# facebookresearch/habitat-lab

Hardware: NVIDIA H100
Metric: DD-PPO learner frames/sec (ResNet18 RGB-D 256x256) (higher is better)
Workload: dtype bf16

## Files before the change

habitat-lab_b200/csrc/elementwise.cu:

```cuda
#include "common.cuh"
#include "wgmma.cuh"
#include <cooperative_groups.h>

namespace hb200 {
namespace cg = cooperative_groups;
using wg::cp_async16;
using wg::cp_async_commit;
using wg::cp_async_wait;
using wg::smem_u32;
void count_launch(int n);

static inline int grid_for(long long n, int bs) {
  long long g = (n + bs - 1) / bs;
  const long long cap = (long long)kNumSMs * 16;
  return (int)(g < 1 ? 1 : (g > cap ? cap : g));
}

template <bool HAS_RGB, bool HAS_DEPTH>
__device__ __forceinline__ void pooled4(const uint8_t* __restrict__ rgb, const float* __restrict__ depth,
                                        size_t row, int H, int W, int py, int px4, float rgb_scale,
                                        float (&out)[4][4]) {
#pragma unroll
  for (int p = 0; p < 4; ++p)
#pragma unroll
    for (int c = 0; c < 4; ++c) out[p][c] = 0.f;
  if (HAS_RGB) {
    const uint8_t* base = rgb + (row * H + 2 * py) * (size_t)W * 3 + (size_t)px4 * 8 * 3;
    uint8_t v[2][24];
#pragma unroll
    for (int r = 0; r < 2; ++r) {
      const uint2* src = reinterpret_cast<const uint2*>(base + (size_t)r * W * 3);
#pragma unroll
      for (int q = 0; q < 3; ++q) {
        const uint2 u = __ldg(src + q);
        *reinterpret_cast<uint2*>(&v[r][q * 8]) = u;
      }
    }
#pragma unroll
    for (int p = 0; p < 4; ++p)
#pragma unroll
      for (int c = 0; c < 3; ++c) {
        float s = __fmul_rn((float)v[0][(2 * p) * 3 + c], rgb_scale);
        s = __fadd_rn(s, __fmul_rn((float)v[0][(2 * p + 1) * 3 + c], rgb_scale));
        s = __fadd_rn(s, __fmul_rn((float)v[1][(2 * p) * 3 + c], rgb_scale));
        s = __fadd_rn(s, __fmul_rn((float)v[1][(2 * p + 1) * 3 + c], rgb_scale));
        out[p][c] = s * 0.25f;
      }
  }
  if (HAS_DEPTH) {
    const int dc = HAS_RGB ? 3 : 0;
    const float* base = depth + (row * H + 2 * py) * (size_t)W + (size_t)px4 * 8;
    float d[2][8];
#pragma unroll
    for (int r = 0; r < 2; ++r) {
      const float4* src = reinterpret_cast<const float4*>(base + (size_t)r * W);
      const float4 a = __ldg(src), b = __ldg(src + 1);
      d[r][0] = a.x; d[r][1] = a.y; d[r][2] = a.z; d[r][3] = a.w;
      d[r][4] = b.x; d[r][5] = b.y; d[r][6] = b.z; d[r][7] = b.w;
    }
#pragma unroll
    for (int p = 0; p < 4; ++p) {
      float s = __fadd_rn(d[0][2 * p], d[0][2 * p + 1]);
      s = __fadd_rn(s, d[1][2 * p]);
      s = __fadd_rn(s, d[1][2 * p + 1]);
      out[p][dc] = s * 0.25f;
    }
  }
}

template <bool HAS_RGB, bool HAS_DEPTH>
__global__ void __launch_bounds__(256)
prep_stats_kernel(const uint8_t* __restrict__ rgb, const float* __restrict__ depth,
                  const int32_t* __restrict__ frame_rows, int B, int H, int W, float rgb_scale,
                  double* __restrict__ stats) {
  __shared__ double red[32];
  const int Hp = H / 2, Wq = W / 8;
  const long long total = (long long)B * Hp * Wq;
  float s[4] = {0, 0, 0, 0}, q[4] = {0, 0, 0, 0};
  for (long long i = blockIdx.x * (long long)blockDim.x + threadIdx.x; i < total;
       i += (long long)gridDim.x * blockDim.x) {
    const int px4 = (int)(i % Wq);
    const long long t = i / Wq;
    const int py = (int)(t % Hp);
    const int f = (int)(t / Hp);
    float o[4][4];
    pooled4<HAS_RGB, HAS_DEPTH>(rgb, depth, (size_t)frame_rows[f], H, W, py, px4, rgb_scale, o);
#pragma unroll
    for (int p = 0; p < 4; ++p)
#pragma unroll
      for (int c = 0; c < 4; ++c) { s[c] += o[p][c]; q[c] = fmaf(o[p][c], o[p][c], q[c]); }
  }
#pragma unroll
  for (int c = 0; c < 4; ++c) {
    const double a = block_sum((double)s[c], red);
    const double b = block_sum((double)q[c], red);
    if (threadIdx.x == 0) { atomicAdd(&stats[c], a); atomicAdd(&stats[8 + c], b); }
  }
  if (blockIdx.x == 0 && threadIdx.x == 0) stats[16] = (double)B;
}

template <bool HAS_RGB, bool HAS_DEPTH, bool S2D>
__global__ void __launch_bounds__(256)
prep_apply_kernel(const uint8_t* __restrict__ rgb, const float* __restrict__ depth,
                  const int32_t* __restrict__ frame_rows, int B, int H, int W, float rgb_scale,
                  const float* __restrict__ scale_shift, act_t* __restrict__ out, grad_t* __restrict__ out2) {
  const int Hp = H / 2, Wq = W / 8;
  const long long total = (long long)B * Hp * Wq;
  float sc[4] = {1, 1, 1, 1}, sh[4] = {0, 0, 0, 0};
  if (scale_shift) {
#pragma unroll
    for (int c = 0; c < 4; ++c) { sc[c] = scale_shift[c]; sh[c] = scale_shift[8 + c]; }
  }
  const int C = (HAS_RGB ? 3 : 0) + (HAS_DEPTH ? 1 : 0);
  for (long long i = blockIdx.x * (long long)blockDim.x + threadIdx.x; i < total;
       i += (long long)gridDim.x * blockDim.x) {
    const int px4 = (int)(i % Wq);
    const long long t = i / Wq;
    const int py = (int)(t % Hp);
    const int f = (int)(t / Hp);
    float o[4][4];
    pooled4<HAS_RGB, HAS_DEPTH>(rgb, depth, (size_t)frame_rows[f], H, W, py, px4, rgb_scale, o);
    if (!S2D) {
      uint4* dst = reinterpret_cast<uint4*>(out + (((size_t)f * Hp + py) * (W / 2) + (size_t)px4 * 4) * 8);
#pragma unroll
      for (int p = 0; p < 4; ++p) {
        float v[8] = {0, 0, 0, 0, 0, 0, 0, 0};
#pragma unroll
        for (int c = 0; c < 4; ++c)
          if (c < C) v[c] = fmaf(o[p][c], sc[c], sh[c]);
        dst[p] = pack8a(v);
        if (out2) reinterpret_cast<uint4*>(out2 + (((size_t)f * Hp + py) * (W / 2) + (size_t)px4 * 4) * 8)[p] = pack8(v);
      }
    } else {
      const int i2 = py >> 1, dy = py & 1;
#pragma unroll
      for (int q = 0; q < 2; ++q) {
        float v[8];
#pragma unroll
        for (int dx = 0; dx < 2; ++dx)
#pragma unroll
          for (int c = 0; c < 4; ++c) v[dx * 4 + c] = (c < C) ? fmaf(o[2 * q + dx][c], sc[c], sh[c]) : 0.f;
        const size_t pix = ((size_t)f * (Hp / 2) + i2) * (W / 4) + (size_t)px4 * 2 + q;
        *reinterpret_cast<uint4*>(out + pix * 16 + dy * 8) = pack8a(v);
        if (out2) *reinterpret_cast<uint4*>(out2 + pix * 16 + dy * 8) = pack8(v);
      }
    }
  }
}

__global__ void prep_finalize_kernel(const double* __restrict__ stats, float* __restrict__ run_mean,
                                     float* __restrict__ run_var, float* __restrict__ run_count,
                                     float* __restrict__ scale_shift, int C, long long pix_per_frame,
                                     int update) {
  const int c = threadIdx.x;
  __shared__ float s_count;
  if (c == 0) s_count = run_count[0];
  __syncthreads();
  if (c < C) {
    float mean = run_mean[c], var = run_var[c];
    if (update) {
      const double frames = stats[16];
      const double n_el = frames * (double)pix_per_frame;
      const double nm = stats[c] / n_el;
      double nv = stats[8 + c] / n_el - nm * nm;
      if (nv < 0) nv = 0;
      const float count = s_count, new_count = (float)frames;
      const float new_mean = (float)nm, new_var = (float)nv;
      const float m_a = var * count, m_b = new_var * new_count;
      const float d = new_mean - mean;
      const float M2 = m_a + m_b + d * d * count * new_count / (count + new_count);
      var = M2 / (count + new_count);
      mean = (count * mean + new_count * new_mean) / (count + new_count);
      run_mean[c] = mean;
      run_var[c] = var;
    }
    const float inv = 1.0f / sqrtf(fmaxf(var, 1e-2f));
    scale_shift[c] = inv;
    scale_shift[8 + c] = -mean * inv;
  } else if (c < 8) {
    scale_shift[c] = 0.f;
    scale_shift[8 + c] = 0.f;
  }
  __syncthreads();
  if (c == 0 && update) run_count[0] = s_count + (float)stats[16];
}

struct GnP {
  const double* stats;
  const float* gamma;
  const float* beta;
  int C, G, lcpg;
  float inv_m, eps;
};

__device__ __forceinline__ void gn_coeffs(const GnP& p, int b, int c0, float (&mu)[8], float (&rs)[8]) {
  int prev = -1;
  float m = 0.f, r = 0.f;
#pragma unroll
  for (int e = 0; e < 8; ++e) {
    const int g = (c0 + e) >> p.lcpg;
    if (g != prev) {
      const double2 st = *reinterpret_cast<const double2*>(p.stats + ((size_t)b * p.G + g) * 2);
      const double md = st.x * (double)p.inv_m;
      m = (float)md;
      const float var = fmaxf((float)(st.y * (double)p.inv_m - md * md), 0.f);
      r = rsqrtf(var + p.eps);
      prev = g;
    }
    mu[e] = m;
    rs[e] = r;
  }
}
__device__ __forceinline__ void load8f(const float* __restrict__ p, float (&f)[8]) {
  const float4 a = __ldg(reinterpret_cast<const float4*>(p));
  const float4 b = __ldg(reinterpret_cast<const float4*>(p) + 1);
  f[0] = a.x; f[1] = a.y; f[2] = a.z; f[3] = a.w; f[4] = b.x; f[5] = b.y; f[6] = b.z; f[7] = b.w;
}

struct GnSlab {
  int b, vec, c0, pix0, pix1, npl, pl;
};
__device__ __forceinline__ GnSlab gn_slab(int C, int hw, int ppb) {
  GnSlab s;
  const int cv = C >> 3;
  const int slabs = (hw + ppb - 1) / ppb;
  s.b = blockIdx.x / slabs;
  const int slab = blockIdx.x - s.b * slabs;
  s.vec = threadIdx.x % cv;
  s.pl = threadIdx.x / cv;
  s.npl = blockDim.x / cv;
  s.c0 = s.vec << 3;
  s.pix0 = slab * ppb;
  s.pix1 = min(hw, s.pix0 + ppb);
  return s;
}

template <int OUT_F32>
__global__ void __launch_bounds__(256)
gn_apply_kernel(const act_t* __restrict__ y, GnP p, void* __restrict__ out, grad_t* __restrict__ out2, int B, int hw,
                int relu, int ppb) {
  const GnSlab t = gn_slab(p.C, hw, ppb);
  const int cv = p.C >> 3;
  float mu[8], rs[8], ga[8], be[8], sc[8], sh[8];
  gn_coeffs(p, t.b, t.c0, mu, rs);
  load8f(p.gamma + t.c0, ga);
  load8f(p.beta + t.c0, be);
#pragma unroll
  for (int e = 0; e < 8; ++e) { sc[e] = rs[e] * ga[e]; sh[e] = fmaf(-mu[e], sc[e], be[e]); }
  for (int pix = t.pix0 + t.pl; pix < t.pix1; pix += t.npl) {
    const size_t i = ((size_t)t.b * hw + pix) * cv + t.vec;
    float x[8];
    unpack8a(reinterpret_cast<const uint4*>(y)[i], x);
#pragma unroll
    for (int e = 0; e < 8; ++e) {
      const float z = fmaf(x[e], sc[e], sh[e]);
      x[e] = relu ? fmaxf(z, 0.f) : z;
    }
    if (OUT_F32 == 1) {
      float4* o = reinterpret_cast<float4*>(out) + 2 * i;
      o[0] = make_float4(x[0], x[1], x[2], x[3]);
      o[1] = make_float4(x[4], x[5], x[6], x[7]);
    } else if (OUT_F32 == 2) {
      float* o = reinterpret_cast<float*>(out) + (size_t)t.b * p.C * hw;
#pragma unroll
      for (int e = 0; e < 8; ++e) o[(size_t)(t.c0 + e) * hw + pix] = x[e];
    } else {
      reinterpret_cast<uint4*>(out)[i] = pack8a(x);
      if (out2) reinterpret_cast<uint4*>(out2)[i] = pack8(x);
    }
  }
}

__global__ void __launch_bounds__(256)
gn_residual_relu_kernel(const act_t* __restrict__ y, GnP p, const act_t* __restrict__ res,
                        GnP rp, int res_is_prenorm, act_t* __restrict__ out, grad_t* __restrict__ out2, int B, int hw,
                        int ppb) {
  const GnSlab t = gn_slab(p.C, hw, ppb);
  const int cv = p.C >> 3;
  float mu[8], rs[8], ga[8], be[8], sc[8], sh[8], rsc[8], rsh[8];
  gn_coeffs(p, t.b, t.c0, mu, rs);
  load8f(p.gamma + t.c0, ga);
  load8f(p.beta + t.c0, be);
#pragma unroll
  for (int e = 0; e < 8; ++e) { sc[e] = rs[e] * ga[e]; sh[e] = fmaf(-mu[e], sc[e], be[e]); rsc[e] = 1.f; rsh[e] = 0.f; }
  if (res_is_prenorm) {
    gn_coeffs(rp, t.b, t.c0, mu, rs);
    load8f(rp.gamma + t.c0, ga);
    load8f(rp.beta + t.c0, be);
#pragma unroll
    for (int e = 0; e < 8; ++e) { rsc[e] = rs[e] * ga[e]; rsh[e] = fmaf(-mu[e], rsc[e], be[e]); }
  }
  for (int pix = t.pix0 + t.pl; pix < t.pix1; pix += t.npl) {
    const size_t i = ((size_t)t.b * hw + pix) * cv + t.vec;
    float x[8], r[8];
    unpack8a(reinterpret_cast<const uint4*>(y)[i], x);
    unpack8a(reinterpret_cast<const uint4*>(res)[i], r);
#pragma unroll
    for (int e = 0; e < 8; ++e) x[e] = fmaxf(fmaf(x[e], sc[e], sh[e]) + fmaf(r[e], rsc[e], rsh[e]), 0.f);
    reinterpret_cast<uint4*>(out)[i] = pack8a(x);
    if (out2) reinterpret_cast<uint4*>(out2)[i] = pack8(x);
  }
}

__global__ void __launch_bounds__(256)
gn_relu_maxpool_kernel(const act_t* __restrict__ y, GnP p, act_t* __restrict__ out, grad_t* __restrict__ out2,
                       uint8_t* __restrict__ argmax, int B, int H, int W) {
  const int cv = p.C >> 3, Ho = (H + 1) / 2, Wo = (W + 1) / 2;
  const long long total = (long long)B * Ho * Wo * cv;
  for (long long i = blockIdx.x * (long long)blockDim.x + threadIdx.x; i < total;
       i += (long long)gridDim.x * blockDim.x) {
    const int c0 = (int)(i % cv) << 3;
    long long t = i / cv;
    const int ox = (int)(t % Wo);
    t /= Wo;
    const int oy = (int)(t % Ho);
    const int b = (int)(t / Ho);
    float mu[8], rs[8], ga[8], be[8], best[8];
    int arg[8];
    gn_coeffs(p, b, c0, mu, rs);
    load8f(p.gamma + c0, ga);
    load8f(p.beta + c0, be);
#pragma unroll
    for (int e = 0; e < 8; ++e) { best[e] = -INFINITY; arg[e] = 0; }
#pragma unroll
    for (int r = 0; r < 3; ++r) {
      const int iy = 2 * oy - 1 + r;
      if (iy < 0 || iy >= H) continue;
#pragma unroll
      for (int s = 0; s < 3; ++s) {
        const int ix = 2 * ox - 1 + s;
        if (ix < 0 || ix >= W) continue;
        float x[8];
        unpack8a(*reinterpret_cast<const uint4*>(y + (((size_t)b * H + iy) * W + ix) * p.C + c0), x);
#pragma unroll
        for (int e = 0; e < 8; ++e) {
          const float z = fmaxf(fmaf((x[e] - mu[e]) * rs[e], ga[e], be[e]), 0.f);
          if (z > best[e]) { best[e] = z; arg[e] = r * 3 + s; }
        }
      }
    }
    reinterpret_cast<uint4*>(out)[i] = pack8a(best);
    if (out2) reinterpret_cast<uint4*>(out2)[i] = pack8(best);
    uint2 a;
    a.x = (uint32_t)arg[0] | ((uint32_t)arg[1] << 8) | ((uint32_t)arg[2] << 16) | ((uint32_t)arg[3] << 24);
    a.y = (uint32_t)arg[4] | ((uint32_t)arg[5] << 8) | ((uint32_t)arg[6] << 16) | ((uint32_t)arg[7] << 24);
    reinterpret_cast<uint2*>(argmax)[i] = a;
  }
}

__global__ void __launch_bounds__(256)
gn_relu_maxpool_slab_kernel(const act_t* __restrict__ y, GnP p, act_t* __restrict__ out, grad_t* __restrict__ out2,
                            uint8_t* __restrict__ argmax, int H, int W, int rows) {
  extern __shared__ __align__(16) uint8_t gsm[];
  uint4* sy = reinterpret_cast<uint4*>(gsm);
  const int cv = p.C >> 3, Ho = H >> 1, Wo = W >> 1, nslab = H / rows;
  const int b = blockIdx.x / nslab, slab = blockIdx.x - b * nslab;
  const int iy0 = slab * rows, yrow = W * cv;
  const int tid = threadIdx.x;
  {
    const int lr0 = iy0 == 0 ? 1 : 0;
    const uint4* gy = reinterpret_cast<const uint4*>(y) + ((size_t)b * H + iy0 - 1 + lr0) * yrow;
    const uint32_t ay = smem_u32(sy) + lr0 * yrow * 16;
    const int n = (rows + 1 - lr0) * yrow;
    for (int i = tid; i < n; i += 256) cp_async16(ay + i * 16, gy + i, true);
    cp_async_commit();
  }
  const int vec = tid % cv, c0 = vec << 3;
  float sg[8], za[8], zd[8];
  {
    float mu[8], rs[8], ga[8], be[8];
    gn_coeffs(p, b, c0, mu, rs);
    load8f(p.gamma + c0, ga);
    load8f(p.beta + c0, be);
#pragma unroll
    for (int e = 0; e < 8; ++e) {
      const float zc = rs[e] * ga[e];
      sg[e] = zc < 0.f ? -1.f : 1.f;
      za[e] = fabsf(zc);
      zd[e] = fmaf(-mu[e], zc, be[e]);
    }
  }
  cp_async_wait<0>();
  __syncthreads();
  const int nout = (rows >> 1) * Wo * cv;
  uint4* o4 = reinterpret_cast<uint4*>(out) + ((size_t)b * Ho + (iy0 >> 1)) * Wo * cv;
  uint4* o4b = out2 ? reinterpret_cast<uint4*>(out2) + ((size_t)b * Ho + (iy0 >> 1)) * Wo * cv : nullptr;
  uint2* a2 = reinterpret_cast<uint2*>(argmax) + ((size_t)b * Ho + (iy0 >> 1)) * Wo * cv;
  for (int it = tid; it < nout; it += 256) {
    const int pos = it / cv, ol = pos / Wo, ox = pos - ol * Wo;
    float best[8];
    int arg[8];
#pragma unroll
    for (int e = 0; e < 8; ++e) { best[e] = -INFINITY; arg[e] = 0; }
#pragma unroll
    for (int r = 0; r < 3; ++r) {
      const int lr = 2 * ol + r;
      if (iy0 + lr < 1) continue;
#pragma unroll
      for (int s = 0; s < 3; ++s) {
        const int ix = 2 * ox - 1 + s;
        if (ix < 0) continue;
        float x[8];
        unpack8a(sy[(lr * W + ix) * cv + vec], x);
#pragma unroll
        for (int e = 0; e < 8; ++e) {
          const float xs = x[e] * sg[e];
          if (xs > best[e]) { best[e] = xs; arg[e] = r * 3 + s; }
        }
      }
    }
    float z[8];
#pragma unroll
    for (int e = 0; e < 8; ++e) z[e] = fmaxf(fmaf(best[e], za[e], zd[e]), 0.f);
    o4[it] = pack8a(z);
    if (o4b) o4b[it] = pack8(z);
    uint2 a;
    a.x = (uint32_t)arg[0] | ((uint32_t)arg[1] << 8) | ((uint32_t)arg[2] << 16) | ((uint32_t)arg[3] << 24);
    a.y = (uint32_t)arg[4] | ((uint32_t)arg[5] << 8) | ((uint32_t)arg[6] << 16) | ((uint32_t)arg[7] << 24);
    a2[it] = a;
  }
}

__global__ void __launch_bounds__(256)
maxpool_bwd_kernel(const grad_t* __restrict__ dout, const uint8_t* __restrict__ argmax,
                   grad_t* __restrict__ dz, int B, int H, int W, int C) {
  const int cv = C >> 3, Ho = (H + 1) / 2, Wo = (W + 1) / 2;
  const long long total = (long long)B * H * W * cv;
  for (long long i = blockIdx.x * (long long)blockDim.x + threadIdx.x; i < total;
       i += (long long)gridDim.x * blockDim.x) {
    const int c0 = (int)(i % cv) << 3;
    long long t = i / cv;
    const int ix = (int)(t % W);
    t /= W;
    const int iy = (int)(t % H);
    const int b = (int)(t / H);
    float acc[8] = {0, 0, 0, 0, 0, 0, 0, 0};
    const int oy_lo = iy >> 1, oy_hi = (iy + 1) >> 1;
    const int ox_lo = ix >> 1, ox_hi = (ix + 1) >> 1;
    for (int oy = oy_lo; oy <= oy_hi; ++oy) {
      if (oy >= Ho) continue;
      const int r = iy - (2 * oy - 1);
      for (int ox = ox_lo; ox <= ox_hi; ++ox) {
        if (ox >= Wo) continue;
        const int s = ix - (2 * ox - 1);
        const int code = r * 3 + s;
        const size_t o = (((size_t)b * Ho + oy) * Wo + ox) * C + c0;
        const uint2 a = *reinterpret_cast<const uint2*>(argmax + o);
        float g[8];
        unpack8(*reinterpret_cast<const uint4*>(dout + o), g);
// ... 1087 lines not shown
  __shared__ float sred[256][9];
  cg::cluster_group cluster = cg::this_cluster();
  const int CS = (int)cluster.num_blocks(), rank = (int)cluster.block_rank();
  const int b = blockIdx.x / CS;
  const int C = p.C, cv = C >> 3, cr = se.cr, tid = threadIdx.x;
  const int pix0 = rank * ppc, pix1 = min(hw, pix0 + ppc);
  const int n = max(pix1 - pix0, 0) * cv;
  const size_t base = ((size_t)b * hw + pix0) * cv;
  const uint4* gy = reinterpret_cast<const uint4*>(y) + base;
  uint4* sy = reinterpret_cast<uint4*>(gsm);
  float* part = reinterpret_cast<float*>(gsm + (staged ? (size_t)ppc * C * 2 : 0));
  float* tot = part + C;
  float* pv = tot + C;
  float* sv = pv + C;
  float* hv = sv + C;
  if (staged) {
    const uint32_t ay = smem_u32(sy);
    for (int i = tid; i < n; i += 256) cp_async16(ay + i * 16, gy + i, true);
    cp_async_commit();
  }
  const uint4* src = staged ? sy : gy;
  const int vec = tid % cv, c0 = vec << 3;
  float zc[8], zd[8], rsc[8], rsh[8];
  {
    float mu[8], rs[8], ga[8], be[8];
    gn_coeffs(p, b, c0, mu, rs);
    load8f(p.gamma + c0, ga);
    load8f(p.beta + c0, be);
#pragma unroll
    for (int e = 0; e < 8; ++e) { zc[e] = rs[e] * ga[e]; zd[e] = fmaf(-mu[e], zc[e], be[e]); rsc[e] = 1.f; rsh[e] = 0.f; }
    if (res_is_prenorm) {
      gn_coeffs(rp, b, c0, mu, rs);
      load8f(rp.gamma + c0, ga);
      load8f(rp.beta + c0, be);
#pragma unroll
      for (int e = 0; e < 8; ++e) { rsc[e] = rs[e] * ga[e]; rsh[e] = fmaf(-mu[e], rsc[e], be[e]); }
    }
  }
  if (staged) cp_async_wait<0>();
  float acc[8];
#pragma unroll
  for (int e = 0; e < 8; ++e) acc[e] = 0.f;
  for (int i = tid; i < n; i += 256) {
    float x[8];
    unpack8a(src[i], x);
#pragma unroll
    for (int e = 0; e < 8; ++e) acc[e] += x[e];
  }
  se_cta_chan_sum(acc, sred, part, C);
  se_cluster_total(cluster, part, tot, C, CS);
  const float inv_hw = 1.f / (float)hw;
  for (int c = tid; c < C; c += 256) {
    float mu, rs;
    gn_chan(p, b, c, mu, rs);
    const float k = rs * p.gamma[c];
    pv[c] = fmaf(tot[c] * inv_hw, k, fmaf(-mu, k, p.beta[c]));
  }
  __syncthreads();
  const int lane = tid & 31, warp = tid >> 5;
  for (int j = warp; j < cr; j += 8) {
    const float* w = se.w1 + (size_t)j * C;
    float t = 0.f;
    for (int c = lane; c < C; c += 32) t = fmaf(__ldg(w + c), pv[c], t);
#pragma unroll
    for (int o = 16; o > 0; o >>= 1) t += __shfl_xor_sync(0xffffffffu, t, o);
    if (lane == 0) hv[j] = fmaxf(t + __ldg(se.b1 + j), 0.f);
  }
  __syncthreads();
  for (int c = tid; c < C; c += 256) {
    const float4* w = reinterpret_cast<const float4*>(se.w2 + (size_t)c * cr);
    float t = __ldg(se.b2 + c);
    for (int j = 0; j < cr; j += 4) {
      const float4 wv = __ldg(w + (j >> 2));
      t = fmaf(wv.x, hv[j], t);
      t = fmaf(wv.y, hv[j + 1], t);
      t = fmaf(wv.z, hv[j + 2], t);
      t = fmaf(wv.w, hv[j + 3], t);
    }
    sv[c] = 1.f / (1.f + expf(-t));
  }
  __syncthreads();
  if (rank == 0) {
    for (int c = tid; c < C; c += 256) {
      se.p[(size_t)b * C + c] = pv[c];
      se.s[(size_t)b * C + c] = sv[c];
    }
    for (int j = tid; j < cr; j += 256) se.h[(size_t)b * cr + j] = hv[j];
  }
  float sc[8];
#pragma unroll
  for (int e = 0; e < 8; ++e) sc[e] = sv[c0 + e];
  const uint4* gr = reinterpret_cast<const uint4*>(res) + base;
  uint4* go = reinterpret_cast<uint4*>(out) + base;
  uint4* go2 = out2 ? reinterpret_cast<uint4*>(out2) + base : nullptr;
  for (int i = tid; i < n; i += 256) {
    float x[8], r[8];
    unpack8a(src[i], x);
    unpack8a(gr[i], r);
#pragma unroll
    for (int e = 0; e < 8; ++e) x[e] = fmaxf(fmaf(sc[e], fmaf(x[e], zc[e], zd[e]), fmaf(r[e], rsc[e], rsh[e])), 0.f);
    go[i] = pack8a(x);
    if (go2) go2[i] = pack8(x);
  }
  asm volatile("barrier.cluster.wait.acquire.aligned;" ::: "memory");
}

__global__ void __launch_bounds__(256)
gn_se_bwd_kernel(const grad_t* __restrict__ g, const act_t* __restrict__ act, const act_t* __restrict__ y, GnP p,
                 SeP se, float* __restrict__ dgamma, float* __restrict__ dbeta, grad_t* __restrict__ dy,
                 grad_t* __restrict__ gz_out, int hw, int ppc, int staged) {
  extern __shared__ __align__(16) uint8_t gsm[];
  __shared__ float sred[256][9];
  cg::cluster_group cluster = cg::this_cluster();
  const int CS = (int)cluster.num_blocks(), rank = (int)cluster.block_rank();
  const int b = blockIdx.x / CS;
  const int C = p.C, G = p.G, cv = C >> 3, cr = se.cr, tid = threadIdx.x;
  const int pix0 = rank * ppc, pix1 = min(hw, pix0 + ppc);
  const int n = max(pix1 - pix0, 0) * cv, ncap = staged ? ppc * cv : 0;
  const size_t base = ((size_t)b * hw + pix0) * cv;
  const uint4* gg = reinterpret_cast<const uint4*>(g) + base;
  const uint4* gy = reinterpret_cast<const uint4*>(y) + base;
  const uint4* ga = reinterpret_cast<const uint4*>(act) + base;
  uint4* sg = reinterpret_cast<uint4*>(gsm);
  uint4* sy = sg + ncap;
  uint4* sa = sy + ncap;
  float* part = reinterpret_cast<float*>(sa + ncap);
  float* tot = part + 3 * C;
  float* av = tot + 3 * C;
  float* dpv = av + C;
  float* t1 = dpv + C;
  float* t2 = t1 + C;
  float* red = t2 + C;
  float* dhv = red + 256;
  float* gS = dhv + cr;
  if (staged) {
    const uint32_t ag = smem_u32(sg), ay = smem_u32(sy), aa = smem_u32(sa);
    for (int i = tid; i < n; i += 256) {
      cp_async16(ag + i * 16, gg + i, true);
      cp_async16(ay + i * 16, gy + i, true);
      cp_async16(aa + i * 16, ga + i, true);
    }
    cp_async_commit();
  }
  const uint4 *srg = staged ? sg : gg, *sry = staged ? sy : gy, *sra = staged ? sa : ga;
  const int vec = tid % cv, c0 = vec << 3;
  if (staged) cp_async_wait<0>();
  {
    float s1[8], s2[8], s3[8];
#pragma unroll
    for (int e = 0; e < 8; ++e) { s1[e] = 0.f; s2[e] = 0.f; s3[e] = 0.f; }
    for (int i = tid; i < n; i += 256) {
      float gv[8], x[8], ac[8];
      unpack8(srg[i], gv);
      unpack8a(sry[i], x);
      unpack8a(sra[i], ac);
#pragma unroll
      for (int e = 0; e < 8; ++e) {
        const float gz = ac[e] > 0.f ? gv[e] : 0.f;
        s1[e] += gz;
        s2[e] = fmaf(gz, x[e], s2[e]);
        s3[e] += x[e];
      }
    }
    se_cta_chan_sum(s1, sred, part, C);
    se_cta_chan_sum(s2, sred, part + C, C);
    se_cta_chan_sum(s3, sred, part + 2 * C, C);
  }
  se_cluster_total(cluster, part, tot, 3 * C, CS);
  const float* sf = se.s_in + (size_t)b * C;
  for (int c = tid; c < C; c += 256) {
    float mu, rs;
    gn_chan(p, b, c, mu, rs);
    const float k = rs * p.gamma[c], kd = fmaf(-mu, k, p.beta[c]);
    const float ds = fmaf(k, tot[C + c], kd * tot[c]);
    const float s = sf[c];
    const float a = ds * s * (1.f - s);
    av[c] = a;
    if (rank == 0) se.a[(size_t)b * C + c] = a;
  }
  __syncthreads();
  {
    const int j = tid % cr, q = tid / cr, per = C / (256 / cr);
    const float* w = se.w2 + j;
    float t = 0.f;
    for (int c = q * per; c < (q + 1) * per; ++c) t = fmaf(__ldg(w + (size_t)c * cr), av[c], t);
    red[tid] = t;
  }
  __syncthreads();
  if (tid < cr) {
    float t = 0.f;
    for (int q = 0; q < 256 / cr; ++q) t += red[q * cr + tid];
    t = se.h_in[(size_t)b * cr + tid] > 0.f ? t : 0.f;
    dhv[tid] = t;
    if (rank == 0) se.dh[(size_t)b * cr + tid] = t;
  }
  __syncthreads();
  const float inv_hw = 1.f / (float)hw;
  for (int c = tid; c < C; c += 256) {
    float dp = 0.f;
    for (int j = 0; j < cr; ++j) dp = fmaf(__ldg(se.w1 + (size_t)j * C + c), dhv[j], dp);
    const float s = sf[c];
    const float ta = fmaf(s, tot[c], dp);
    const float tx = fmaf(s, tot[C + c], dp * inv_hw * tot[2 * C + c]);
    float mu, rs;
    gn_chan(p, b, c, mu, rs);
    const float tb = rs * (tx - mu * ta);
    dpv[c] = dp * inv_hw;
    t1[c] = ta;
    t2[c] = tb;
    if (rank == 0) {
      dbeta[(size_t)b * C + c] = ta;
      dgamma[(size_t)b * C + c] = tb;
    }
  }
  __syncthreads();
  const int cpg = 1 << p.lcpg;
  for (int gi = tid; gi < G; gi += 256) {
    float s1 = 0.f, s2 = 0.f;
    for (int c = gi * cpg; c < (gi + 1) * cpg; ++c) {
      const float gm = p.gamma[c];
      s1 = fmaf(gm, t1[c], s1);
      s2 = fmaf(gm, t2[c], s2);
    }
    gS[gi] = s1;
    gS[G + gi] = s2;
  }
  __syncthreads();
  float zc[8], c2[8], c3[8], sc[8], dq[8];
  {
    float mu[8], rs[8], gm[8];
    gn_coeffs(p, b, c0, mu, rs);
    load8f(p.gamma + c0, gm);
#pragma unroll
    for (int e = 0; e < 8; ++e) {
      const int gi = (c0 + e) >> p.lcpg;
      const float k2 = rs[e] * p.inv_m * gS[gi], k3 = rs[e] * p.inv_m * gS[G + gi];
      zc[e] = rs[e] * gm[e];
      c3[e] = -rs[e] * k3;
      c2[e] = fmaf(mu[e] * rs[e], k3, -k2);
      sc[e] = sf[c0 + e];
      dq[e] = dpv[c0 + e];
    }
  }
  uint4* od = reinterpret_cast<uint4*>(dy) + base;
  uint4* oz = gz_out ? reinterpret_cast<uint4*>(gz_out) + base : nullptr;
  for (int i = tid; i < n; i += 256) {
    float gv[8], x[8], ac[8], gz[8], o[8];
    unpack8(srg[i], gv);
    unpack8a(sry[i], x);
    unpack8a(sra[i], ac);
#pragma unroll
    for (int e = 0; e < 8; ++e) {
      gz[e] = ac[e] > 0.f ? gv[e] : 0.f;
      o[e] = fmaf(zc[e], fmaf(sc[e], gz[e], dq[e]), fmaf(x[e], c3[e], c2[e]));
    }
    od[i] = pack8(o);
    if (oz) oz[i] = pack8(gz);
  }
  asm volatile("barrier.cluster.wait.acquire.aligned;" ::: "memory");
}

static int se_launch(const void* kern, int batch, int hw, int C, int ntens, size_t extra, cudaStream_t st,
                     cudaLaunchConfig_t* cfg, cudaLaunchAttribute* at, int* ppc, int* staged) {
  int cs = 1;
  size_t slice = 0;
  for (;; cs *= 2) {
    *ppc = (hw + cs - 1) / cs;
    slice = (size_t)ntens * *ppc * C * 2;
    if (slice <= 48 * 1024 || cs == 8) break;
  }
  *staged = slice + extra <= 200 * 1024 ? 1 : 0;
  const size_t smem = (*staged ? slice : 0) + extra;
  HB_CUDA(cudaFuncSetAttribute(kern, cudaFuncAttributeMaxDynamicSharedMemorySize, (int)smem));
  *cfg = {};
  cfg->gridDim = dim3((unsigned)batch * cs);
  cfg->blockDim = dim3(256);
  cfg->dynamicSmemBytes = smem;
  cfg->stream = st;
  at[0].id = cudaLaunchAttributeClusterDimension;
  at[0].val.clusterDim.x = cs; at[0].val.clusterDim.y = 1; at[0].val.clusterDim.z = 1;
  cfg->attrs = at;
  cfg->numAttrs = 1;
  return HB200_OK;
}

static int se_check(int C, int cr) {
  HB_CHECK_ARG(C / 8 >= 1 && C / 8 <= 256 && 256 % (C / 8) == 0, "gn_se: C/8 = %d must divide 256", C / 8);
  HB_CHECK_ARG(cr >= 4 && cr % 4 == 0 && 256 % cr == 0 && C % (256 / cr) == 0,
               "gn_se: reduced width %d must be a multiple of 4 dividing 256 (and 256/%d must divide C = %d)", cr, cr, C);
  return HB200_OK;
}

}

using namespace hb200;

static int prep_check(const uint8_t* rgb, const float* depth, const int32_t* rows, int B, int H, int W,
                      int c_rgb, int c_depth) {
  HB_CHECK_ARG(rows && B > 0, "prep: bad args");
  HB_CHECK_ARG((c_rgb == 3 && rgb) || (c_rgb == 0), "prep: c_rgb must be 0 or 3");
  HB_CHECK_ARG((c_depth == 1 && depth) || (c_depth == 0), "prep: c_depth must be 0 or 1");
  HB_CHECK_ARG(c_rgb + c_depth > 0, "prep: no visual channels");
  HB_CHECK_ARG(H % 2 == 0 && W % 8 == 0, "prep: H must be even and W a multiple of 8 (got %dx%d)", H, W);
  return HB200_OK;
}

extern "C" int hb200_prep_stats(const uint8_t* rgb, const float* depth, const int32_t* frame_rows,
                                int batch, int height, int width, int c_rgb, int c_depth,
                                float rgb_scale, double* stats_acc, hb200_stream_t stream) {
  int rc = prep_check(rgb, depth, frame_rows, batch, height, width, c_rgb, c_depth);
  if (rc) return rc;
  HB_CHECK_ARG(stats_acc, "prep_stats: null stats");
  cudaStream_t st = (cudaStream_t)stream;
  HB_CUDA(cudaMemsetAsync(stats_acc, 0, 17 * sizeof(double), st));
  const long long total = (long long)batch * (height / 2) * (width / 8);
  const int grid = grid_for(total, 256);
  if (c_rgb && c_depth) prep_stats_kernel<true, true><<<grid, 256, 0, st>>>(rgb, depth, frame_rows, batch, height, width, rgb_scale, stats_acc);
  else if (c_rgb) prep_stats_kernel<true, false><<<grid, 256, 0, st>>>(rgb, depth, frame_rows, batch, height, width, rgb_scale, stats_acc);
  else prep_stats_kernel<false, true><<<grid, 256, 0, st>>>(rgb, depth, frame_rows, batch, height, width, rgb_scale, stats_acc);
  HB_LAUNCH_OK();
  count_launch(1);
  return HB200_OK;
}

extern "C" int hb200_prep_finalize(const double* stats_acc, float* run_mean, float* run_var,
                                   float* run_count, float* scale_shift, int channels,
                                   long long pixels_per_frame, int update, hb200_stream_t stream) {
  HB_CHECK_ARG(stats_acc && run_mean && run_var && run_count && scale_shift, "prep_finalize: null pointer");
  HB_CHECK_ARG(channels > 0 && channels <= 8, "prep_finalize: channels must be 1..8");
  prep_finalize_kernel<<<1, 32, 0, (cudaStream_t)stream>>>(stats_acc, run_mean, run_var, run_count,
                                                            scale_shift, channels, pixels_per_frame, update);
  HB_LAUNCH_OK();
  count_launch(1);
  return HB200_OK;
}

extern "C" int hb200_prep_apply(const uint8_t* rgb, const float* depth, const int32_t* frame_rows,
                                int batch, int height, int width, int c_rgb, int c_depth,
                                float rgb_scale, const float* scale_shift, hb200_f16* out, hb200_bf16* out_bf16,
                                int s2d, hb200_stream_t stream) {
  int rc = prep_check(rgb, depth, frame_rows, batch, height, width, c_rgb, c_depth);
  if (rc) return rc;
  HB_CHECK_ARG(out, "prep_apply: null out");
  cudaStream_t st = (cudaStream_t)stream;
  const long long total = (long long)batch * (height / 2) * (width / 8);
  const int grid = grid_for(total, 256);
  act_t* o = (act_t*)out;
  grad_t* o2 = (grad_t*)out_bf16;
  HB_CHECK_ARG(!s2d || (height % 4 == 0), "prep_apply: s2d needs H %% 4 == 0");
#define HB_PREP(R, D)                                                                                              \
  if (s2d) prep_apply_kernel<R, D, true><<<grid, 256, 0, st>>>(rgb, depth, frame_rows, batch, height, width, rgb_scale, scale_shift, o, o2); \
  else prep_apply_kernel<R, D, false><<<grid, 256, 0, st>>>(rgb, depth, frame_rows, batch, height, width, rgb_scale, scale_shift, o, o2)
  if (c_rgb && c_depth) { HB_PREP(true, true); }
  else if (c_rgb) { HB_PREP(true, false); }
  else { HB_PREP(false, true); }
#undef HB_PREP
  HB_LAUNCH_OK();
  count_launch(1);
  return HB200_OK;
}

extern "C" int hb200_gn_apply(const hb200_f16* y, const double* stats, const float* gamma,
                              const float* beta, void* out, hb200_bf16* out_bf16, int out_f32, int batch, int hw,
                              int channels, int groups, float eps, int relu, hb200_stream_t stream) {
  GnP p;
  int rc = make_gn(p, stats, gamma, beta, channels, groups, hw, eps);
  if (rc) return rc;
  HB_CHECK_ARG(y && out, "gn_apply: null pointer");
  HB_CHECK_ARG(!out_bf16 || out_f32 == 0, "gn_apply: the bf16 twin accompanies the fp16 output only");
  grad_t* o2 = (grad_t*)out_bf16;
  int ppb = 0, grid = 0;
  rc = gn_slab_launch(channels, hw, batch, &ppb, &grid);
  if (rc) return rc;
  if (out_f32 == 1)
    gn_apply_kernel<1><<<grid, 256, 0, (cudaStream_t)stream>>>((const act_t*)y, p, out, o2, batch, hw, relu, ppb);
  else if (out_f32 == 2)
    gn_apply_kernel<2><<<grid, 256, 0, (cudaStream_t)stream>>>((const act_t*)y, p, out, o2, batch, hw, relu, ppb);
  else
    gn_apply_kernel<0><<<grid, 256, 0, (cudaStream_t)stream>>>((const act_t*)y, p, out, o2, batch, hw, relu, ppb);
  HB_LAUNCH_OK();
  count_launch(1);
  return HB200_OK;
}

extern "C" int hb200_gn_residual_relu(const hb200_f16* y, const double* stats, const float* gamma,
                                      const float* beta, const hb200_f16* res, const double* res_stats,
                                      const float* res_gamma, const float* res_beta, hb200_f16* out,
                                      hb200_bf16* out_bf16, int batch, int hw, int channels, int groups, float eps,
                                      hb200_stream_t stream) {
  GnP p, rp;
  int rc = make_gn(p, stats, gamma, beta, channels, groups, hw, eps);
  if (rc) return rc;
  HB_CHECK_ARG(y && res && out, "gn_residual_relu: null pointer");
  rp = p;
  if (res_stats) {
    rc = make_gn(rp, res_stats, res_gamma, res_beta, channels, groups, hw, eps);
    if (rc) return rc;
  }
  int ppb = 0, grid = 0;
  rc = gn_slab_launch(channels, hw, batch, &ppb, &grid);
  if (rc) return rc;
  gn_residual_relu_kernel<<<grid, 256, 0, (cudaStream_t)stream>>>(
      (const act_t*)y, p, (const act_t*)res, rp, res_stats ? 1 : 0, (act_t*)out, (grad_t*)out_bf16, batch, hw, ppb);
  HB_LAUNCH_OK();
  count_launch(1);
  return HB200_OK;
}

extern "C" int hb200_gn_relu_maxpool(const hb200_f16* y, const double* stats, const float* gamma,
                                     const float* beta, hb200_f16* out, hb200_bf16* out_bf16, uint8_t* argmax,
                                     int batch, int h, int w, int channels, int groups, float eps,
                                     hb200_stream_t stream) {
  GnP p;
  int rc = make_gn(p, stats, gamma, beta, channels, groups, h * w, eps);
  if (rc) return rc;
  HB_CHECK_ARG(y && out && argmax && h > 0 && w > 0, "gn_relu_maxpool: bad args");
  if (h % 2 == 0 && w % 2 == 0) {
    const int cv = channels / 8;
    int rows = 0;
    for (int r = 8; r >= 2; r -= 2)
      if (h % r == 0 && (size_t)(r + 1) * w * channels * 2 <= 64 * 1024) { rows = r; break; }
    if (rows && cv <= 32 && 256 % cv == 0) {
      const size_t smem = (size_t)(rows + 1) * w * channels * 2;
      auto kern = gn_relu_maxpool_slab_kernel;
      HB_CUDA(cudaFuncSetAttribute(kern, cudaFuncAttributeMaxDynamicSharedMemorySize, (int)smem));
      kern<<<batch * (h / rows), 256, smem, (cudaStream_t)stream>>>((const act_t*)y, p, (act_t*)out,
                                                                    (grad_t*)out_bf16, argmax, h, w, rows);
      HB_LAUNCH_OK();
      count_launch(1);
      return HB200_OK;
    }
  }
  const long long total = (long long)batch * ((h + 1) / 2) * ((w + 1) / 2) * (channels / 8);
  gn_relu_maxpool_kernel<<<grid_for(total, 256), 256, 0, (cudaStream_t)stream>>>(
      (const act_t*)y, p, (act_t*)out, (grad_t*)out_bf16, argmax, batch, h, w);
  HB_LAUNCH_OK();
  count_launch(1);
  return HB200_OK;
}

extern "C" int hb200_maxpool_bwd(const hb200_bf16* dout, const uint8_t* argmax, hb200_bf16* dz,
                                 int batch, int h, int w, int channels, hb200_stream_t stream) {
  HB_CHECK_ARG(dout && argmax && dz && channels % 8 == 0 && h > 0 && w > 0, "maxpool_bwd: bad args");
  const long long total = (long long)batch * h * w * (channels / 8);
  maxpool_bwd_kernel<<<grid_for(total, 256), 256, 0, (cudaStream_t)stream>>>(
      (const grad_t*)dout, argmax, (grad_t*)dz, batch, h, w, channels);
  HB_LAUNCH_OK();
  count_launch(1);
  return HB200_OK;
}

extern "C" int hb200_gn_bwd_reduce(const hb200_bf16* g, const hb200_bf16* act, const hb200_bf16* y,
                                   const double* stats, const float* gamma, const float* beta,
                                   float* sums, float* dgamma, float* dbeta, int batch, int hw,
                                   int channels, int groups, float eps, int mask_mode,
                                   hb200_stream_t stream) {
  GnP p;
  int rc = make_gn(p, stats, gamma, beta, channels, groups, hw, eps);
  if (rc) return rc;
  HB_CHECK_ARG(g && y && sums && dgamma && dbeta, "gn_bwd_reduce: null pointer");
  HB_CHECK_ARG(mask_mode >= 0 && mask_mode <= 2 && (mask_mode != 2 || act), "gn_bwd_reduce: bad mask_mode");
  HB_CHECK_ARG(channels <= 2048 && 256 % (channels / 8) == 0, "gn_bwd_reduce: C/8 must divide 256");
  cudaStream_t st = (cudaStream_t)stream;
  HB_CUDA(cudaMemsetAsync(sums, 0, sizeof(float) * 2 * (size_t)batch * groups, st));
  const int npl = 256 / (channels / 8);
  int ppb = npl * 16;
  if (ppb > hw) ppb = hw;
  const int slabs = (hw + ppb - 1) / ppb;
  gn_bwd_reduce_kernel<<<batch * slabs, 256, 0, st>>>((const grad_t*)g, (const act_t*)act,
                                                      (const act_t*)y, p, sums, dgamma, dbeta,
                                                      batch, hw, ppb, mask_mode);
  HB_LAUNCH_OK();
  count_launch(1);
  return HB200_OK;
}

extern "C" int hb200_gn_bwd_apply(const hb200_bf16* g, const hb200_bf16* act, const hb200_bf16* y,
                                  const double* stats, const float* gamma, const float* beta,
                                  const float* sums, hb200_bf16* dy, hb200_bf16* gz_out, int batch,
                                  int hw, int channels, int groups, float eps, int mask_mode,
                                  hb200_stream_t stream) {
  GnP p;
  int rc = make_gn(p, stats, gamma, beta, channels, groups, hw, eps);
  if (rc) return rc;
  HB_CHECK_ARG(g && y && sums && dy, "gn_bwd_apply: null pointer");
  HB_CHECK_ARG(mask_mode >= 0 && mask_mode <= 2 && (mask_mode != 2 || act), "gn_bwd_apply: bad mask_mode");
  int ppb = 0, grid = 0;
  rc = gn_slab_launch(channels, hw, batch, &ppb, &grid);
  if (rc) return rc;
  gn_bwd_apply_kernel<<<grid, 256, 0, (cudaStream_t)stream>>>(
      (const grad_t*)g, (const act_t*)act, (const act_t*)y, p, sums,
      (grad_t*)dy, (grad_t*)gz_out, batch, hw, mask_mode, ppb);
  HB_LAUNCH_OK();
  count_launch(1);
  return HB200_OK;
}

extern "C" int hb200_bf16_to_f32(const hb200_bf16* x, float* out, long long n, hb200_stream_t stream) {
  HB_CHECK_ARG(x && out && n > 0 && n % 8 == 0, "bf16_to_f32: n must be a positive multiple of 8");
  bf16_to_f32_kernel<<<grid_for(n / 8, 256), 256, 0, (cudaStream_t)stream>>>((const __nv_bfloat16*)x, out, n / 8);
  HB_LAUNCH_OK();
  count_launch(1);
  return HB200_OK;
}
extern "C" int hb200_f16_to_bf16(const hb200_f16* x, hb200_bf16* out, long long n, hb200_stream_t stream) {
  HB_CHECK_ARG(x && out && n % 8 == 0, "f16_to_bf16: n must be a multiple of 8");
  f16_to_bf16_kernel<<<grid_for(n / 8, 256), 256, 0, (cudaStream_t)stream>>>((const act_t*)x, (grad_t*)out, n / 8);
  HB_LAUNCH_OK();
  count_launch(1);
  return HB200_OK;
}

extern "C" int hb200_f32_to_bf16(const float* x, hb200_bf16* out, long long n, hb200_stream_t stream) {
  HB_CHECK_ARG(x && out && n > 0 && n % 8 == 0, "f32_to_bf16: n must be a positive multiple of 8");
  f32_to_bf16_kernel<<<grid_for(n / 8, 256), 256, 0, (cudaStream_t)stream>>>(x, (__nv_bfloat16*)out, n / 8);
  HB_LAUNCH_OK();
  count_launch(1);
  return HB200_OK;
}

extern "C" int hb200_embed_fwd(const float* goal, const int64_t* prev_actions, const uint8_t* masks,
                               const int32_t* frame_rows, const float* w_tgt, const float* b_tgt,
                               const float* emb_table, float* out, int ld, int col0, int batch,
                               hb200_stream_t stream) {
  HB_CHECK_ARG(goal && prev_actions && masks && frame_rows && w_tgt && b_tgt && emb_table && out && batch > 0,
               "embed_fwd: bad args");
  embed_fwd_kernel<<<grid_for((long long)batch * 64, 256), 256, 0, (cudaStream_t)stream>>>(
      goal, prev_actions, masks, frame_rows, w_tgt, b_tgt, emb_table, out, ld, col0, batch);
  HB_LAUNCH_OK();
  count_launch(1);
  return HB200_OK;
}
extern "C" int hb200_embed_bwd(const float* goal, const int64_t* prev_actions, const uint8_t* masks,
                               const int32_t* frame_rows, const float* d_out, int ld, int col0,
                               int batch, int n_emb, float* d_w_tgt, float* d_b_tgt, float* d_emb,
                               hb200_stream_t stream) {
  HB_CHECK_ARG(goal && prev_actions && masks && frame_rows && d_out && d_w_tgt && d_b_tgt && d_emb && batch > 0,
               "embed_bwd: bad args");
  HB_CHECK_ARG(n_emb > 0 && n_emb <= 64, "embed_bwd: n_emb out of range");
  cudaStream_t st = (cudaStream_t)stream;
  const int nacc = 128 + n_emb * 32, nparts = cdiv(batch, kEmbedFrames);
  float* parts = nullptr;
  int* tickets = nullptr;
  int rc = stream_workspace(st, (size_t)(nparts + kReduceChunks) * nacc, 0, &parts, &tickets);
  if (rc) return rc;
  float* tmp = parts + (size_t)nparts * nacc;
  embed_bwd_kernel<<<dim3(cdiv(nacc, 128), nparts), 128, 0, st>>>(goal, prev_actions, masks, frame_rows, d_out, ld,
                                                                   col0, batch, n_emb, parts);
  HB_LAUNCH_OK();
  count_launch(1);
  rc = reduce_partials(parts, nparts, nacc, 96, d_w_tgt, tmp, st);
  if (!rc) rc = reduce_partials(parts + 96, nparts, nacc, 32, d_b_tgt, tmp, st);
  if (!rc) rc = reduce_partials(parts + 128, nparts, nacc, (long long)n_emb * 32, d_emb, tmp, st);
  return rc;
}

extern "C" int hb200_sensor_linear_fwd(const float* x, int in_dim, const int32_t* frame_rows, int batch, int transform,
                                       const float* w, const float* b, float* out, int ld, int col0, int out_dim,
                                       hb200_stream_t stream) {
  HB_CHECK_ARG(x && frame_rows && out && batch > 0 && in_dim >= 1 && in_dim <= 8, "sensor_linear_fwd: bad args");
  HB_CHECK_ARG(transform >= 0 && transform <= 3 && out_dim >= 1 && out_dim <= 64, "sensor_linear_fwd: bad transform / width");
  HB_CHECK_ARG((w && b) || (!w && transform == 0 && out_dim == in_dim), "sensor_linear_fwd: raw copy needs identity features");
  sensor_linear_fwd_kernel<<<grid_for((long long)batch * out_dim, 256), 256, 0, (cudaStream_t)stream>>>(
      x, in_dim, frame_rows, batch, transform, w, b, out, ld, col0, out_dim);
  HB_LAUNCH_OK();
  count_launch(1);
  return HB200_OK;
}

extern "C" int hb200_sensor_linear_bwd(const float* x, int in_dim, const int32_t* frame_rows, int batch, int transform,
                                       const float* d_out, int ld, int col0, int out_dim, float* d_w, float* d_b,
                                       hb200_stream_t stream) {
  HB_CHECK_ARG(x && frame_rows && d_out && d_w && d_b && batch > 0 && in_dim >= 1 && in_dim <= 8, "sensor_linear_bwd: bad args");
  HB_CHECK_ARG(transform >= 0 && transform <= 3 && out_dim >= 1 && out_dim <= 64, "sensor_linear_bwd: bad transform / width");
  const int nf = transform == 1 ? 3 : (transform == 2 ? 4 : (transform == 3 ? 2 : in_dim));
  const int nacc = out_dim * (nf + 1), nparts = cdiv(batch, kEmbedFrames);
  HB_CHECK_ARG(nparts <= 65535, "sensor_linear_bwd: batch %d exceeds %d frames", batch, 65535 * kEmbedFrames);
  cudaStream_t st = (cudaStream_t)stream;
  float* parts = nullptr;
  int* tickets = nullptr;
  int rc = stream_workspace(st, (size_t)(nparts + kReduceChunks) * nacc, 0, &parts, &tickets);
  if (rc) return rc;
  float* tmp = parts + (size_t)nparts * nacc;
  sensor_linear_bwd_kernel<<<dim3(cdiv(nacc, 128), nparts), 128, 0, st>>>(x, in_dim, frame_rows, batch, transform, d_out,
                                                                          ld, col0, out_dim, nf, parts);
  HB_LAUNCH_OK();
  count_launch(1);
  rc = reduce_partials(parts, nparts, nacc, (long long)out_dim * nf, d_w, tmp, st);
  if (!rc) rc = reduce_partials(parts + (size_t)out_dim * nf, nparts, nacc, out_dim, d_b, tmp, st);
  return rc;
}

extern "C" int hb200_index_embed_fwd(const int64_t* idx, const int32_t* frame_rows, const uint8_t* masks, int batch,
                                     int table_rows, const float* table, int width, float* out, int ld, int col0,
                                     hb200_stream_t stream) {
  HB_CHECK_ARG(idx && table && out && batch > 0 && table_rows > 0 && width > 0, "index_embed_fwd: bad args");
  index_embed_fwd_kernel<<<grid_for((long long)batch * width, 256), 256, 0, (cudaStream_t)stream>>>(
      idx, frame_rows, masks, batch, table_rows, table, width, out, ld, col0);
  HB_LAUNCH_OK();
  count_launch(1);
  return HB200_OK;
}

extern "C" int hb200_index_embed_bwd(const int64_t* idx, const int32_t* frame_rows, const uint8_t* masks, int batch,
                                     int table_rows, int width, const float* d_out, int ld, int col0, float* d_table,
                                     hb200_stream_t stream) {
  HB_CHECK_ARG(idx && d_out && d_table && batch > 0 && table_rows > 0 && width > 0, "index_embed_bwd: bad args");
  const long long nacc = (long long)table_rows * width;
  const int nparts = cdiv(batch, kEmbedFrames);
  HB_CHECK_ARG(nparts <= 65535, "index_embed_bwd: batch %d exceeds %d frames", batch, 65535 * kEmbedFrames);
  cudaStream_t st = (cudaStream_t)stream;
  float* parts = nullptr;
  int* tickets = nullptr;
  const int rc = stream_workspace(st, (size_t)(nparts + kReduceChunks) * nacc, 0, &parts, &tickets);
  if (rc) return rc;
  index_embed_bwd_kernel<<<dim3(cdiv(nacc, 128), nparts), 128, 0, st>>>(idx, frame_rows, masks, batch, table_rows, width,
                                                                        d_out, ld, col0, parts);
  HB_LAUNCH_OK();
  count_launch(1);
  return reduce_partials(parts, nparts, nacc, nacc, d_table, parts + (size_t)nparts * nacc, st);
}

extern "C" int hb200_prep_generic(const void* const* h_srcs, const int* h_dtypes, const int* h_channels,
                                  const float* h_scales, int n_srcs, const int32_t* frame_rows, int batch, int height,
                                  int width, const float* scale_shift, hb200_f16* out, hb200_bf16* out_bf16,
                                  double* stats_acc, hb200_stream_t stream) {
  HB_CHECK_ARG(h_srcs && h_dtypes && h_channels && h_scales && n_srcs >= 1 && n_srcs <= 4, "prep_generic: 1..4 sources");
  HB_CHECK_ARG(frame_rows && batch > 0 && height >= 2 && width >= 2, "prep_generic: bad shape");
  HB_CHECK_ARG((stats_acc != nullptr) != (out != nullptr), "prep_generic: pass either stats_acc (statistics pass) or out (apply pass)");
  PrepSrcs src;
  int ctot = 0;
  for (int k = 0; k < 4; ++k) { src.ptr[k] = nullptr; src.dtype[k] = 0; src.channels[k] = 0; src.scale[k] = 1.f; }
  for (int k = 0; k < n_srcs; ++k) {
    HB_CHECK_ARG(h_srcs[k] && h_dtypes[k] >= 0 && h_dtypes[k] <= 2 && h_channels[k] >= 1, "prep_generic: bad source %d", k);
    src.ptr[k] = h_srcs[k]; src.dtype[k] = h_dtypes[k]; src.channels[k] = h_channels[k]; src.scale[k] = h_scales[k];
    ctot += h_channels[k];
  }
  HB_CHECK_ARG(ctot <= 8, "prep_generic: at most 8 input channels (got %d)", ctot);
  src.n = n_srcs;
  cudaStream_t st = (cudaStream_t)stream;
  const long long total = (long long)batch * (height / 2) * (width / 2);
  const int grid = grid_for(total, 256);
  if (stats_acc) {
    HB_CUDA(cudaMemsetAsync(stats_acc, 0, 17 * sizeof(double), st));
    prep_generic_kernel<true><<<grid, 256, 0, st>>>(src, frame_rows, batch, height, width, nullptr, nullptr, nullptr, stats_acc);
  } else {
    prep_generic_kernel<false><<<grid, 256, 0, st>>>(src, frame_rows, batch, height, width, scale_shift, (act_t*)out,
                                                     (grad_t*)out_bf16, nullptr);
  }
  HB_LAUNCH_OK();
  count_launch(1);
  return HB200_OK;
}


extern "C" int hb200_rnn_shift_mask(const float* h_seq, const float* h0, long long h0_row_stride,
                                    const uint8_t* masks, float* h_in, int t_steps, int n, int hidden,
                                    hb200_stream_t stream) {
  HB_CHECK_ARG(h_seq && h0 && masks && h_in && t_steps > 0 && n > 0 && hidden > 0, "rnn_shift_mask: bad args");
  const long long total = (long long)t_steps * n * hidden;
  rnn_shift_mask_kernel<<<grid_for(total, 256), 256, 0, (cudaStream_t)stream>>>(h_seq, h0, h0_row_stride, masks,
                                                                                 h_in, t_steps, n, hidden);
// ... 311 lines not shown
```

Measured before the change: 57680.

## Restructure prep_apply into per-frame row bands with paired coalesced stores

The input preprocessing kernel now launches one block per band of pooled rows per frame instead of a capped grid-stride loop. This removes per-element div/mod index math and repeated frame_rows lookups. In S2D mode each thread pools two rows, so it writes full 32-element output pixels. Neighbouring lanes then swap halves with warp shuffles so each pair writes contiguous 16-byte chunks, giving better coalesced stores for both the fp16 and bf16 outputs. It adds 16-byte alignment checks and shuffle overhead, and grid size now grows with the batch.

```diff
diff --git a/habitat-lab_b200/csrc/elementwise.cu b/habitat-lab_b200/csrc/elementwise.cu
--- a/habitat-lab_b200/csrc/elementwise.cu
+++ b/habitat-lab_b200/csrc/elementwise.cu
@@ -99,52 +99,70 @@
   if (blockIdx.x == 0 && threadIdx.x == 0) stats[16] = (double)B;
 }
 
+constexpr int kPrepThreads = 256;
+
+template <typename T>
+__device__ __forceinline__ void prep_store_pair(T* __restrict__ out, size_t e, const uint4 (&u)[4], bool ok,
+                                                bool partner_ok) {
+  const bool odd = threadIdx.x & 1;
+  uint4 r[2];
+#pragma unroll
+  for (int k = 0; k < 2; ++k) {
+    const uint4 x = odd ? u[2 * k] : u[2 * k + 1];
+    r[k].x = __shfl_xor_sync(0xffffffffu, x.x, 1);
+    r[k].y = __shfl_xor_sync(0xffffffffu, x.y, 1);
+    r[k].z = __shfl_xor_sync(0xffffffffu, x.z, 1);
+    r[k].w = __shfl_xor_sync(0xffffffffu, x.w, 1);
+  }
+  if (ok && partner_ok) {
+    T* d = out + e - (odd ? 32 : 0) + (odd ? 8 : 0);
+    const uint4 v[4] = {odd ? r[0] : u[0], odd ? r[1] : u[2], odd ? u[1] : r[0], odd ? u[3] : r[1]};
+#pragma unroll
+    for (int k = 0; k < 4; ++k) *reinterpret_cast<uint4*>(d + 16 * k) = v[k];
+  } else if (ok) {
+#pragma unroll
+    for (int k = 0; k < 4; ++k) reinterpret_cast<uint4*>(out + e)[k] = u[k];
+  }
+}
+
 template <bool HAS_RGB, bool HAS_DEPTH, bool S2D>
-__global__ void __launch_bounds__(256)
+__global__ void __launch_bounds__(kPrepThreads)
 prep_apply_kernel(const uint8_t* __restrict__ rgb, const float* __restrict__ depth,
-                  const int32_t* __restrict__ frame_rows, int B, int H, int W, float rgb_scale,
+                  const int32_t* __restrict__ frame_rows, int H, int W, int rp, float rgb_scale,
                   const float* __restrict__ scale_shift, act_t* __restrict__ out, grad_t* __restrict__ out2) {
-  const int Hp = H / 2, Wq = W / 8;
-  const long long total = (long long)B * Hp * Wq;
+  constexpr int C = (HAS_RGB ? 3 : 0) + (HAS_DEPTH ? 1 : 0);
+  constexpr int PR = S2D ? 2 : 1;
   float sc[4] = {1, 1, 1, 1}, sh[4] = {0, 0, 0, 0};
   if (scale_shift) {
 #pragma unroll
     for (int c = 0; c < 4; ++c) { sc[c] = scale_shift[c]; sh[c] = scale_shift[8 + c]; }
   }
-  const int C = (HAS_RGB ? 3 : 0) + (HAS_DEPTH ? 1 : 0);
-  for (long long i = blockIdx.x * (long long)blockDim.x + threadIdx.x; i < total;
-       i += (long long)gridDim.x * blockDim.x) {
-    const int px4 = (int)(i % Wq);
-    const long long t = i / Wq;
-    const int py = (int)(t % Hp);
-    const int f = (int)(t / Hp);
-    float o[4][4];
-    pooled4<HAS_RGB, HAS_DEPTH>(rgb, depth, (size_t)frame_rows[f], H, W, py, px4, rgb_scale, o);
-    if (!S2D) {
-      uint4* dst = reinterpret_cast<uint4*>(out + (((size_t)f * Hp + py) * (W / 2) + (size_t)px4 * 4) * 8);
-#pragma unroll
-      for (int p = 0; p < 4; ++p) {
-        float v[8] = {0, 0, 0, 0, 0, 0, 0, 0};
-#pragma unroll
-        for (int c = 0; c < 4; ++c)
-          if (c < C) v[c] = fmaf(o[p][c], sc[c], sh[c]);
-        dst[p] = pack8a(v);
-        if (out2) reinterpret_cast<uint4*>(out2 + (((size_t)f * Hp + py) * (W / 2) + (size_t)px4 * 4) * 8)[p] = pack8(v);
+  const int Hp = H / 2, Wq = W / 8, nb = (Hp + rp - 1) / rp;
+  const int f = blockIdx.x / nb, p0 = (blockIdx.x - f * nb) * rp, n = min(rp, Hp - p0) / PR * Wq;
+  const size_t row = (size_t)frame_rows[f];
+  const size_t base = ((size_t)f * Hp + p0) * W * (S2D ? 2 : 4);
+  for (int i0 = threadIdx.x & ~31; i0 < n; i0 += kPrepThreads) {
+    const int li = i0 + (threadIdx.x & 31), i = min(li, n - 1);
+    const int r = i / Wq, px4 = i - r * Wq;
+    float o[PR][4][4];
+#pragma unroll
+    for (int dy = 0; dy < PR; ++dy)
+      pooled4<HAS_RGB, HAS_DEPTH>(rgb, depth, row, H, W, p0 + r * PR + dy, px4, rgb_scale, o[dy]);
+    uint4 ua[4], ub[4];
+#pragma unroll
+    for (int k = 0; k < 4; ++k) {
+      float v[8];
+#pragma unroll
+      for (int t = 0; t < 8; ++t) {
+        const int dy = S2D ? (k & 1) : 0, p = S2D ? (k >> 1) * 2 + t / 4 : k, c = S2D ? t % 4 : t;
+        v[t] = (c < C) ? fmaf(o[dy][p][c % 4], sc[c % 4], sh[c % 4]) : 0.f;
       }
-    } else {
-      const int i2 = py >> 1, dy = py & 1;
-#pragma unroll
-      for (int q = 0; q < 2; ++q) {
-        float v[8];
-#pragma unroll
-        for (int dx = 0; dx < 2; ++dx)
-#pragma unroll
-          for (int c = 0; c < 4; ++c) v[dx * 4 + c] = (c < C) ? fmaf(o[2 * q + dx][c], sc[c], sh[c]) : 0.f;
-        const size_t pix = ((size_t)f * (Hp / 2) + i2) * (W / 4) + (size_t)px4 * 2 + q;
-        *reinterpret_cast<uint4*>(out + pix * 16 + dy * 8) = pack8a(v);
-        if (out2) *reinterpret_cast<uint4*>(out2 + pix * 16 + dy * 8) = pack8(v);
-      }
-    }
+      ua[k] = pack8a(v);
+      ub[k] = pack8(v);
+    }
+    const size_t e = base + (size_t)i * 32;
+    prep_store_pair(out, e, ua, li < n, (li ^ 1) < n);
+    if (out2) prep_store_pair(out2, e, ub, li < n, (li ^ 1) < n);
   }
 }
 
@@ -1838,6 +1856,23 @@
   HB_CHECK_ARG((c_depth == 1 && depth) || (c_depth == 0), "prep: c_depth must be 0 or 1");
   HB_CHECK_ARG(c_rgb + c_depth > 0, "prep: no visual channels");
   HB_CHECK_ARG(H % 2 == 0 && W % 8 == 0, "prep: H must be even and W a multiple of 8 (got %dx%d)", H, W);
+  HB_CHECK_ARG((((uintptr_t)rgb | (uintptr_t)depth) & 15) == 0, "prep: rgb / depth must be 16-byte aligned");
+  return HB200_OK;
+}
+
+static int prep_band_rows(int H, int W, int rows_per_thread) {
+  int rp = rows_per_thread * kPrepThreads / (W / 8);
+  rp = (rp < H / 2 ? rp : H / 2) & ~1;
+  return rp > 2 ? rp : 2;
+}
+
+template <typename K, typename... A>
+static int prep_launch(K kernel, int batch, int H, int rp, cudaStream_t st, A... args) {
+  const long long grid = (long long)batch * ((H / 2 + rp - 1) / rp);
+  HB_CHECK_ARG(grid < (1ll << 31), "prep: batch %d too large", batch);
+  kernel<<<(unsigned)grid, kPrepThreads, 0, st>>>(args...);
+  HB_LAUNCH_OK();
+  count_launch(1);
   return HB200_OK;
 }
 
@@ -1879,21 +1914,18 @@
   if (rc) return rc;
   HB_CHECK_ARG(out, "prep_apply: null out");
   cudaStream_t st = (cudaStream_t)stream;
-  const long long total = (long long)batch * (height / 2) * (width / 8);
-  const int grid = grid_for(total, 256);
+  HB_CHECK_ARG((((uintptr_t)out | (uintptr_t)out_bf16) & 15) == 0, "prep_apply: outputs must be 16-byte aligned");
   act_t* o = (act_t*)out;
   grad_t* o2 = (grad_t*)out_bf16;
   HB_CHECK_ARG(!s2d || (height % 4 == 0), "prep_apply: s2d needs H %% 4 == 0");
-#define HB_PREP(R, D)                                                                                              \
-  if (s2d) prep_apply_kernel<R, D, true><<<grid, 256, 0, st>>>(rgb, depth, frame_rows, batch, height, width, rgb_scale, scale_shift, o, o2); \
-  else prep_apply_kernel<R, D, false><<<grid, 256, 0, st>>>(rgb, depth, frame_rows, batch, height, width, rgb_scale, scale_shift, o, o2)
-  if (c_rgb && c_depth) { HB_PREP(true, true); }
-  else if (c_rgb) { HB_PREP(true, false); }
-  else { HB_PREP(false, true); }
+  const int rp = prep_band_rows(height, width, s2d ? 2 : 1);
+#define HB_PREP(R, D, S)                                                                                           \
+  prep_launch(prep_apply_kernel<R, D, S>, batch, height, rp, st, rgb, depth, frame_rows, height, width, rp,       \
+              rgb_scale, scale_shift, o, o2)
+  if (c_rgb && c_depth) return s2d ? HB_PREP(true, true, true) : HB_PREP(true, true, false);
+  if (c_rgb) return s2d ? HB_PREP(true, false, true) : HB_PREP(true, false, false);
+  return s2d ? HB_PREP(false, true, true) : HB_PREP(false, true, false);
 #undef HB_PREP
-  HB_LAUNCH_OK();
-  count_launch(1);
-  return HB200_OK;
 }
 
 extern "C" int hb200_gn_apply(const hb200_f16* y, const double* stats, const float* gamma,
```

After: 59220, median of 6. 2.7% higher.
